# declare-lab/tango

Measured on NVIDIA H100. Metric: audio_seconds_per_second, higher is better.
Workload: dtype bf16

## Files before the change

### tango_b200/csrc/attention.cu

```cuda
#include "tng_ptx.cuh"
#include "tng_internal.h"

namespace tng {

constexpr int FA_BM = 128;
constexpr int FA_BN = 64;
constexpr int FA_QCHUNK = FA_BM * 128;
constexpr int FA_KCHUNK = FA_BN * 128;
constexpr int FA_THREADS = 256;

struct AttnParams {
  int Lq, Lk;
  int q_col0, q_lo_off, k_col0, k_lo_off, v_col0, v_lo_off;
  const float* kbias;
  __nv_bfloat16* out;
  long long ld_o;
  int split_off;
  float scale_log2e;
};

template <int D, int DV, int NSPLIT, int NBUF>
struct FlashCfg {
  static constexpr int Q_BYTES = NSPLIT * (D / 64) * FA_QCHUNK;
  static constexpr int K_BYTES = NSPLIT * (D / 64) * FA_KCHUNK;
  static constexpr int V_BYTES = NSPLIT * (DV / 64) * FA_KCHUNK;
  static constexpr int SMEM_BYTES = Q_BYTES + NBUF * (K_BYTES + V_BYTES) + 128;
  static_assert((1 + 4 * NBUF) * 8 <= 128, "the mbarriers fit the 128 bytes after the tiles");
  static_assert(SMEM_BYTES <= 227 * 1024, "an H100 CTA has at most 227 KB of dynamic shared memory");
};

template <int D, int DV, int NSPLIT, int NBUF>
__global__ void __launch_bounds__(FA_THREADS, (D == 64 && NSPLIT == 1) ? 2 : 1)
flash_attention_kernel(const __grid_constant__ CUtensorMap qmap, const __grid_constant__ CUtensorMap kmap,
                       const __grid_constant__ CUtensorMap vmap, const __grid_constant__ AttnParams p) {
  using Cfg = FlashCfg<D, DV, NSPLIT, NBUF>;
  constexpr int DC = D / 64, NV = DV / 64;
  extern __shared__ __align__(1024) uint8_t smem[];
  uint8_t* sQ = smem;
  uint8_t* sK = sQ + Cfg::Q_BYTES;
  uint8_t* sV = sK + NBUF * Cfg::K_BYTES;
  uint64_t* bars = reinterpret_cast<uint64_t*>(sV + NBUF * Cfg::V_BYTES);
  uint64_t* bar_q = bars;
  uint64_t* full_k = bars + 1;
  uint64_t* full_v = bars + 1 + NBUF;
  uint64_t* empty_k = bars + 1 + 2 * NBUF;
  uint64_t* empty_v = bars + 1 + 3 * NBUF;

  const int tid = threadIdx.x;
  const int warp = tid >> 5;
  const int lane = tid & 31;
  const int wg = warp >> 2;
  const int q0 = blockIdx.x * FA_BM;
  const int b = blockIdx.z;
  const int n_tiles = (p.Lk + FA_BN - 1) / FA_BN;
  const int qk_col = blockIdx.y * (DV == D ? D : 0);
  const int vo_col = blockIdx.y * DV;

  auto load_k = [&](int t) {
    const int buf = t % NBUF;
    mbar_arrive_expect_tx(&full_k[buf], Cfg::K_BYTES);
#pragma unroll
    for (int s = 0; s < NSPLIT; ++s)
#pragma unroll
      for (int c = 0; c < DC; ++c)
        tma_load_3d(sK + buf * Cfg::K_BYTES + (s * DC + c) * FA_KCHUNK, &kmap, &full_k[buf],
                    p.k_col0 + s * p.k_lo_off + qk_col + 64 * c, t * FA_BN, b);
  };
  auto load_v = [&](int t) {
    const int buf = t % NBUF;
    mbar_arrive_expect_tx(&full_v[buf], Cfg::V_BYTES);
#pragma unroll
    for (int s = 0; s < NSPLIT; ++s)
#pragma unroll
      for (int c = 0; c < NV; ++c)
        tma_load_3d(sV + buf * Cfg::V_BYTES + (s * NV + c) * FA_KCHUNK, &vmap, &full_v[buf],
                    p.v_col0 + s * p.v_lo_off + vo_col + 64 * c, t * FA_BN, b);
  };

  if (tid == 0) {
    if ((smem_u32(smem) & 1023u) != 0) __trap();
    tma_prefetch_desc(&qmap);
    tma_prefetch_desc(&kmap);
    tma_prefetch_desc(&vmap);
    mbar_init(bar_q, 1);
    for (int i = 0; i < NBUF; ++i) {
      mbar_init(&full_k[i], 1);
      mbar_init(&full_v[i], 1);
      mbar_init(&empty_k[i], 2);
      mbar_init(&empty_v[i], 2);
    }
    fence_mbar_init();
    mbar_arrive_expect_tx(bar_q, Cfg::Q_BYTES);
#pragma unroll
    for (int s = 0; s < NSPLIT; ++s)
#pragma unroll
      for (int c = 0; c < DC; ++c)
        tma_load_3d(sQ + (s * DC + c) * FA_QCHUNK, &qmap, bar_q, p.q_col0 + s * p.q_lo_off + qk_col + 64 * c, q0, b);
    for (int t = 0; t < NBUF && t < n_tiles; ++t) { load_k(t); load_v(t); }
  }
  __syncthreads();

  constexpr int NT = (NSPLIT == 1) ? 1 : 3;
  const int qsel[3] = {0, 1, 0}, ksel[3] = {0, 0, 1};
  const uint32_t q_base = smem_u32(sQ) + wg * (64 * 128);
  const uint32_t k_base = smem_u32(sK), v_base = smem_u32(sV);
  const float sc = p.scale_log2e;
  constexpr float LOG2E = 1.4426950408889634f;
  const float* kb = p.kbias ? p.kbias + static_cast<long long>(b) * p.Lk : nullptr;
  const int t4 = lane & 3;
  float m_run[2] = {-INFINITY, -INFINITY};
  float l_run[2] = {0.f, 0.f};
  float o[NV][32];
#pragma unroll
  for (int n = 0; n < NV; ++n)
#pragma unroll
    for (int i = 0; i < 32; ++i) o[n][i] = 0.f;

  mbar_wait(bar_q, 0);
  for (int t = 0; t < n_tiles; ++t) {
    const int buf = t % NBUF;
    const uint32_t ph = (t / NBUF) & 1;
    if (NBUF > 1 && tid == 0 && t >= 1 && t - 1 + NBUF < n_tiles) {
      const int pb = (t - 1) % NBUF;
      const uint32_t pph = ((t - 1) / NBUF) & 1;
      mbar_wait(&empty_k[pb], pph);
      load_k(t - 1 + NBUF);
      mbar_wait(&empty_v[pb], pph);
      load_v(t - 1 + NBUF);
    }
    float s[32];
    mbar_wait(&full_k[buf], ph);
    fence_regs(s);
    wgmma_fence();
#pragma unroll
    for (int u = 0; u < NT; ++u) {
#pragma unroll
      for (int c = 0; c < DC; ++c) {
        const uint64_t qd = wgmma_desc_sw128(q_base + (qsel[u] * DC + c) * FA_QCHUNK, 16, 1024);
        const uint64_t kd = wgmma_desc_sw128(k_base + buf * Cfg::K_BYTES + (ksel[u] * DC + c) * FA_KCHUNK, 16, 1024);
#pragma unroll
        for (int k = 0; k < 4; ++k) wgmma_ss<64>(s, qd + 2 * k, kd + 2 * k, (u > 0 || c > 0 || k > 0) ? 1u : 0u);
      }
    }
    wgmma_commit();
    wgmma_wait<0>();
    fence_regs(s);
    if ((tid & 127) == 0) mbar_arrive(&empty_k[buf]);
    if (NBUF == 1 && tid == 0 && t + 1 < n_tiles) {
      mbar_wait(&empty_k[buf], ph);
      load_k(t + 1);
    }

    const int kv0 = t * FA_BN;
    const bool tail = D == 64 && ((kb != nullptr) || (kv0 + FA_BN > p.Lk));
#pragma unroll
    for (int j = 0; j < 8; ++j) {
#pragma unroll
      for (int e = 0; e < 2; ++e) {
        float bias = 0.f;
        if (tail) {
          const int kv = kv0 + 8 * j + 2 * t4 + e;
          bias = kv < p.Lk ? (kb ? __ldg(kb + kv) * LOG2E : 0.f) : -INFINITY;
        }
        s[4 * j + e] = fmaf(s[4 * j + e], sc, bias);
        s[4 * j + 2 + e] = fmaf(s[4 * j + 2 + e], sc, bias);
      }
    }
    float corr[2];
    softmax_step(s, m_run, l_run, corr);
#pragma unroll
    for (int n = 0; n < NV; ++n) rescale_rows(o[n], corr);
    uint32_t pa[NSPLIT][4][4];
    pack_p(pa[0], s);
    if constexpr (NSPLIT == 2) pack_p<true>(pa[1], s);

    mbar_wait(&full_v[buf], ph);
#pragma unroll
    for (int n = 0; n < NV; ++n) fence_regs(o[n]);
    wgmma_fence();
#pragma unroll
    for (int u = 0; u < NT; ++u) {
      const int ps = (NSPLIT == 2 && u == 1) ? NSPLIT - 1 : 0;
#pragma unroll
      for (int n = 0; n < NV; ++n) {
        const uint64_t vd = wgmma_desc_sw128(v_base + buf * Cfg::V_BYTES + (ksel[u] * NV + n) * FA_KCHUNK, 1024, 1024);
#pragma unroll
        for (int kk = 0; kk < FA_BN / 16; ++kk) wgmma_rs_n64_tb(o[n], pa[ps][kk], vd + ((kk * 2048) >> 4), 1u);
      }
    }
    wgmma_commit();
    wgmma_wait<0>();
#pragma unroll
    for (int n = 0; n < NV; ++n) fence_regs(o[n]);
    if ((tid & 127) == 0) mbar_arrive(&empty_v[buf]);
    if (NBUF == 1 && tid == 0 && t + 1 < n_tiles) {
      mbar_wait(&empty_v[buf], ph);
      load_v(t + 1);
    }
  }

  float inv[2];
  softmax_inv(l_run, inv);
#pragma unroll
  for (int h = 0; h < 2; ++h) {
    const int q = q0 + 64 * wg + 16 * (warp & 3) + (lane >> 2) + 8 * h;
    if (q >= p.Lq) continue;
    __nv_bfloat16* op = p.out + (static_cast<long long>(b) * p.Lq + q) * p.ld_o + vo_col + 2 * t4;
#pragma unroll
    for (int n = 0; n < NV; ++n)
#pragma unroll
      for (int j = 0; j < 8; ++j) {
        const float y0 = o[n][4 * j + 2 * h] * inv[h], y1 = o[n][4 * j + 2 * h + 1] * inv[h];
        *reinterpret_cast<uint32_t*>(op + 64 * n + 8 * j) = pack_bf16(y0, y1);
        if (p.split_off > 0)
          *reinterpret_cast<uint32_t*>(op + p.split_off + 64 * n + 8 * j) = pack_bf16_lo(y0, y1);
      }
  }
}

template <int D, int DV, int NSPLIT, int NBUF>
static int launch_flash(const void* q, long long ld_q, const void* k, long long ld_k, const void* v, long long ld_v,
                        int batch, int ny, const AttnParams& p, const char* what, void* stream) {
  constexpr int smem_bytes = FlashCfg<D, DV, NSPLIT, NBUF>::SMEM_BYTES;
  CUtensorMap qm, km, vm;
  int rc = encode_tmap_rows_bf16(&qm, q, ld_q, p.Lq, batch, FA_BM);
  if (!rc) rc = encode_tmap_rows_bf16(&km, k, ld_k, p.Lk, batch, FA_BN);
  if (!rc) rc = encode_tmap_rows_bf16(&vm, v, ld_v, p.Lk, batch, FA_BN);
  if (!rc) rc = set_max_dynamic_smem<flash_attention_kernel<D, DV, NSPLIT, NBUF>>(smem_bytes, what);
  if (rc) return rc;
  dim3 grid((p.Lq + FA_BM - 1) / FA_BM, ny, batch);
  flash_attention_kernel<D, DV, NSPLIT, NBUF>
      <<<grid, FA_THREADS, smem_bytes, reinterpret_cast<cudaStream_t>(stream)>>>(qm, km, vm, p);
  return check_launch(what);
}

}

using namespace tng;

extern "C" int tng_attention(const tng_attn_desc* d, void* stream) {
  if (!d || !d->q || !d->k || !d->v || !d->out) return set_error(TNG_EINVAL, "attention: null argument");
  if (d->nsplit != 1 && d->nsplit != 2) return set_error(TNG_EINVAL, "attention: nsplit=%d", d->nsplit);
  if (d->batch <= 0 || d->heads <= 0 || d->Lq <= 0 || d->Lk <= 0) return set_error(TNG_EINVAL, "attention: bad sizes");
  if (d->scale <= 0.f) return set_error(TNG_EINVAL, "attention: scale must be positive");
  if (d->ld_o % 8 || d->split_off % 8 || (reinterpret_cast<uintptr_t>(d->out) & 15))
    return set_error(TNG_EINVAL, "attention: output must allow 16-byte stores");
  AttnParams p;
  p.Lq = d->Lq; p.Lk = d->Lk;
  p.q_col0 = d->q_col0; p.q_lo_off = d->q_lo_off;
  p.k_col0 = d->k_col0; p.k_lo_off = d->k_lo_off;
  p.v_col0 = d->v_col0; p.v_lo_off = d->v_lo_off;
  p.kbias = d->kbias;
  p.out = reinterpret_cast<__nv_bfloat16*>(d->out);
  p.ld_o = d->ld_o; p.split_off = d->split_off;
  p.scale_log2e = d->scale * 1.4426950408889634f;
  if (d->nsplit == 2)
    return launch_flash<64, 64, 2, 3>(d->q, d->ld_q, d->k, d->ld_k, d->v, d->ld_v, d->batch, d->heads, p, "attention",
                                      stream);
  return launch_flash<64, 64, 1, 3>(d->q, d->ld_q, d->k, d->ld_k, d->v, d->ld_v, d->batch, d->heads, p, "attention",
                                    stream);
}

extern "C" int tng_attention_wide(const void* q, int64_t ld_q, int32_t q_col0, const void* k, int64_t ld_k, int32_t k_col0,
                                  const void* v, int64_t ld_v, int32_t v_col0, void* out, int64_t ld_o, int32_t batch,
                                  int32_t L, int32_t dim, float scale, void* stream) {
  if (!q || !k || !v || !out || batch <= 0 || L <= 0) return set_error(TNG_EINVAL, "attention_wide: bad argument");
  if (dim != 512) return set_error(TNG_EINVAL, "attention_wide: head width %d unsupported (512 only)", dim);
  if (L % FA_BM != 0) return set_error(TNG_EINVAL, "attention_wide: L = %d must be a multiple of %d", L, FA_BM);
  if (scale <= 0.f) return set_error(TNG_EINVAL, "attention_wide: scale must be positive");
  if (ld_o % 8 || (reinterpret_cast<uintptr_t>(out) & 15)) return set_error(TNG_EINVAL, "attention_wide: output must allow 16-byte stores");
  AttnParams p{};
  p.Lq = L; p.Lk = L;
  p.q_col0 = q_col0; p.k_col0 = k_col0; p.v_col0 = v_col0;
  p.out = reinterpret_cast<__nv_bfloat16*>(out);
  p.ld_o = ld_o;
  p.scale_log2e = scale * 1.4426950408889634f;
  return launch_flash<512, 256, 1, 1>(q, ld_q, k, ld_k, v, ld_v, batch, 2, p, "attention_wide", stream);
}
```

### tango_b200/csrc/tng_ptx.cuh

```cuda
#pragma once
#include <cuda_runtime.h>
#include <cuda_bf16.h>
#include <cuda.h>
#include <stdint.h>
#include <stdio.h>
#include "../../include/tango_b200.h"

namespace tng {

#ifndef TNG_SPIN_LIMIT
#define TNG_SPIN_LIMIT (1u << 28)
#endif

__device__ __forceinline__ uint32_t smem_u32(const void* p) {
  return static_cast<uint32_t>(__cvta_generic_to_shared(p));
}

__device__ __forceinline__ void mbar_init(uint64_t* bar, uint32_t count) {
  asm volatile("mbarrier.init.shared::cta.b64 [%0], %1;" ::"r"(smem_u32(bar)), "r"(count));
}
__device__ __forceinline__ void fence_mbar_init() {
  asm volatile("fence.mbarrier_init.release.cluster;" ::: "memory");
}
__device__ __forceinline__ void mbar_arrive_expect_tx(uint64_t* bar, uint32_t bytes) {
  asm volatile("mbarrier.arrive.expect_tx.shared::cta.b64 _, [%0], %1;" ::"r"(smem_u32(bar)), "r"(bytes)
               : "memory");
}
__device__ __forceinline__ void mbar_arrive(uint64_t* bar) {
  asm volatile("mbarrier.arrive.shared::cta.b64 _, [%0];" ::"r"(smem_u32(bar)) : "memory");
}
__device__ __forceinline__ void mbar_arrive_if(uint64_t* bar, bool pred) {
  asm volatile(
      "{\n\t.reg .pred p;\n\tsetp.ne.b32 p, %1, 0;\n\t@p mbarrier.arrive.shared::cta.b64 _, [%0];\n\t}"
      ::"r"(smem_u32(bar)), "r"((uint32_t)pred) : "memory");
}
template <int N>
__device__ __forceinline__ void setmaxnreg_dec() { asm volatile("setmaxnreg.dec.sync.aligned.u32 %0;" ::"n"(N)); }
template <int N>
__device__ __forceinline__ void setmaxnreg_inc() { asm volatile("setmaxnreg.inc.sync.aligned.u32 %0;" ::"n"(N)); }
__device__ __forceinline__ uint32_t mbar_try_wait(uint64_t* bar, uint32_t parity) {
  uint32_t ok;
  asm volatile(
      "{\n\t"
      ".reg .pred P;\n\t"
      "mbarrier.try_wait.parity.shared::cta.b64 P, [%1], %2;\n\t"
      "selp.u32 %0, 1, 0, P;\n\t"
      "}\n"
      : "=r"(ok)
      : "r"(smem_u32(bar)), "r"(parity)
      : "memory");
  return ok;
}
__device__ __forceinline__ void mbar_wait(uint64_t* bar, uint32_t parity) {
  uint32_t spins = 0;
  while (!mbar_try_wait(bar, parity)) {
    if (++spins > TNG_SPIN_LIMIT) __trap();
  }
}

__device__ __forceinline__ void tma_prefetch_desc(const CUtensorMap* m) {
  asm volatile("prefetch.tensormap [%0];" ::"l"(reinterpret_cast<uint64_t>(m)) : "memory");
}
__device__ __forceinline__ void tma_load_2d(void* smem, const CUtensorMap* m, uint64_t* bar, int c0, int c1) {
  asm volatile(
      "cp.async.bulk.tensor.2d.shared::cluster.global.mbarrier::complete_tx::bytes [%0], [%1, {%3, %4}], [%2];"
      ::"r"(smem_u32(smem)), "l"(reinterpret_cast<uint64_t>(m)), "r"(smem_u32(bar)), "r"(c0), "r"(c1)
      : "memory");
}
__device__ __forceinline__ void tma_load_3d(void* smem, const CUtensorMap* m, uint64_t* bar, int c0, int c1,
                                            int c2) {
  asm volatile(
      "cp.async.bulk.tensor.3d.shared::cluster.global.mbarrier::complete_tx::bytes [%0], [%1, {%3, %4, %5}], [%2];"
      ::"r"(smem_u32(smem)), "l"(reinterpret_cast<uint64_t>(m)), "r"(smem_u32(bar)), "r"(c0), "r"(c1), "r"(c2)
      : "memory");
}
__device__ __forceinline__ void tma_load_4d(void* smem, const CUtensorMap* m, uint64_t* bar, int c0, int c1,
                                            int c2, int c3) {
  asm volatile(
      "cp.async.bulk.tensor.4d.shared::cluster.global.mbarrier::complete_tx::bytes [%0], [%1, {%3, %4, %5, %6}], "
      "[%2];" ::"r"(smem_u32(smem)),
      "l"(reinterpret_cast<uint64_t>(m)), "r"(smem_u32(bar)), "r"(c0), "r"(c1), "r"(c2), "r"(c3)
      : "memory");
}

__device__ __forceinline__ void wgmma_fence() { asm volatile("wgmma.fence.sync.aligned;" ::: "memory"); }
__device__ __forceinline__ void wgmma_commit() { asm volatile("wgmma.commit_group.sync.aligned;" ::: "memory"); }
template <int N>
__device__ __forceinline__ void wgmma_wait() {
  asm volatile("wgmma.wait_group.sync.aligned %0;" ::"n"(N) : "memory");
}
template <int R>
__device__ __forceinline__ void fence_regs(float (&d)[R]) {
#pragma unroll
  for (int i = 0; i < R; ++i) asm volatile("" : "+f"(d[i])::"memory");
}

__device__ __forceinline__ uint64_t wgmma_desc_sw128(uint32_t saddr, uint32_t lbo_bytes, uint32_t sbo_bytes) {
  uint64_t d = 0;
  d |= static_cast<uint64_t>((saddr & 0x3FFFF) >> 4);
  d |= static_cast<uint64_t>((lbo_bytes >> 4) & 0x3FFF) << 16;
  d |= static_cast<uint64_t>((sbo_bytes >> 4) & 0x3FFF) << 32;
  d |= static_cast<uint64_t>(1) << 62;
  return d;
}

template <int N>
__device__ __forceinline__ void wgmma_ss(float (&d)[N / 2], uint64_t a_desc, uint64_t b_desc, uint32_t scale_d);

template <>
__device__ __forceinline__ void wgmma_ss<32>(float (&d)[16], uint64_t a_desc, uint64_t b_desc, uint32_t scale_d) {
  asm volatile(
      "{\n\t.reg .pred p;\n\tsetp.ne.b32 p, %18, 0;\n\t"
      "wgmma.mma_async.sync.aligned.m64n32k16.f32.bf16.bf16 {%0, %1, %2, %3, %4, %5, %6, %7, %8, %9, %10, %11, %12, %13, %14, %15}, %16, %17, p, 1, 1, 0, 0;\n\t}\n"
      : "+f"(d[0]), "+f"(d[1]), "+f"(d[2]), "+f"(d[3]), "+f"(d[4]), "+f"(d[5]), "+f"(d[6]), "+f"(d[7]),
        "+f"(d[8]), "+f"(d[9]), "+f"(d[10]), "+f"(d[11]), "+f"(d[12]), "+f"(d[13]), "+f"(d[14]), "+f"(d[15])
      : "l"(a_desc), "l"(b_desc), "r"(scale_d));
}

template <>
__device__ __forceinline__ void wgmma_ss<64>(float (&d)[32], uint64_t a_desc, uint64_t b_desc, uint32_t scale_d) {
  asm volatile(
      "{\n\t.reg .pred p;\n\tsetp.ne.b32 p, %34, 0;\n\t"
      "wgmma.mma_async.sync.aligned.m64n64k16.f32.bf16.bf16 {%0, %1, %2, %3, %4, %5, %6, %7, %8, %9, %10, %11, %12, %13, %14, %15, %16, %17, %18, %19, %20, %21, %22, %23, %24, %25, %26, %27, %28, %29, %30, %31}, %32, %33, p, 1, 1, 0, 0;\n\t}\n"
      : "+f"(d[0]), "+f"(d[1]), "+f"(d[2]), "+f"(d[3]), "+f"(d[4]), "+f"(d[5]), "+f"(d[6]), "+f"(d[7]),
        "+f"(d[8]), "+f"(d[9]), "+f"(d[10]), "+f"(d[11]), "+f"(d[12]), "+f"(d[13]), "+f"(d[14]), "+f"(d[15]),
        "+f"(d[16]), "+f"(d[17]), "+f"(d[18]), "+f"(d[19]), "+f"(d[20]), "+f"(d[21]), "+f"(d[22]), "+f"(d[23]),
        "+f"(d[24]), "+f"(d[25]), "+f"(d[26]), "+f"(d[27]), "+f"(d[28]), "+f"(d[29]), "+f"(d[30]), "+f"(d[31])
      : "l"(a_desc), "l"(b_desc), "r"(scale_d));
}

template <>
__device__ __forceinline__ void wgmma_ss<128>(float (&d)[64], uint64_t a_desc, uint64_t b_desc, uint32_t scale_d) {
  asm volatile(
      "{\n\t.reg .pred p;\n\tsetp.ne.b32 p, %66, 0;\n\t"
      "wgmma.mma_async.sync.aligned.m64n128k16.f32.bf16.bf16 {%0, %1, %2, %3, %4, %5, %6, %7, %8, %9, %10, %11, %12, %13, %14, %15, %16, %17, %18, %19, %20, %21, %22, %23, %24, %25, %26, %27, %28, %29, %30, %31, %32, %33, %34, %35, %36, %37, %38, %39, %40, %41, %42, %43, %44, %45, %46, %47, %48, %49, %50, %51, %52, %53, %54, %55, %56, %57, %58, %59, %60, %61, %62, %63}, %64, %65, p, 1, 1, 0, 0;\n\t}\n"
      : "+f"(d[0]), "+f"(d[1]), "+f"(d[2]), "+f"(d[3]), "+f"(d[4]), "+f"(d[5]), "+f"(d[6]), "+f"(d[7]),
        "+f"(d[8]), "+f"(d[9]), "+f"(d[10]), "+f"(d[11]), "+f"(d[12]), "+f"(d[13]), "+f"(d[14]), "+f"(d[15]),
        "+f"(d[16]), "+f"(d[17]), "+f"(d[18]), "+f"(d[19]), "+f"(d[20]), "+f"(d[21]), "+f"(d[22]), "+f"(d[23]),
        "+f"(d[24]), "+f"(d[25]), "+f"(d[26]), "+f"(d[27]), "+f"(d[28]), "+f"(d[29]), "+f"(d[30]), "+f"(d[31]),
        "+f"(d[32]), "+f"(d[33]), "+f"(d[34]), "+f"(d[35]), "+f"(d[36]), "+f"(d[37]), "+f"(d[38]), "+f"(d[39]),
        "+f"(d[40]), "+f"(d[41]), "+f"(d[42]), "+f"(d[43]), "+f"(d[44]), "+f"(d[45]), "+f"(d[46]), "+f"(d[47]),
        "+f"(d[48]), "+f"(d[49]), "+f"(d[50]), "+f"(d[51]), "+f"(d[52]), "+f"(d[53]), "+f"(d[54]), "+f"(d[55]),
        "+f"(d[56]), "+f"(d[57]), "+f"(d[58]), "+f"(d[59]), "+f"(d[60]), "+f"(d[61]), "+f"(d[62]), "+f"(d[63])
      : "l"(a_desc), "l"(b_desc), "r"(scale_d));
}

template <>
__device__ __forceinline__ void wgmma_ss<160>(float (&d)[80], uint64_t a_desc, uint64_t b_desc, uint32_t scale_d) {
  asm volatile(
      "{\n\t.reg .pred p;\n\tsetp.ne.b32 p, %82, 0;\n\t"
      "wgmma.mma_async.sync.aligned.m64n160k16.f32.bf16.bf16 {%0, %1, %2, %3, %4, %5, %6, %7, %8, %9, %10, %11, %12, %13, %14, %15, %16, %17, %18, %19, %20, %21, %22, %23, %24, %25, %26, %27, %28, %29, %30, %31, %32, %33, %34, %35, %36, %37, %38, %39, %40, %41, %42, %43, %44, %45, %46, %47, %48, %49, %50, %51, %52, %53, %54, %55, %56, %57, %58, %59, %60, %61, %62, %63, %64, %65, %66, %67, %68, %69, %70, %71, %72, %73, %74, %75, %76, %77, %78, %79}, %80, %81, p, 1, 1, 0, 0;\n\t}\n"
      : "+f"(d[0]), "+f"(d[1]), "+f"(d[2]), "+f"(d[3]), "+f"(d[4]), "+f"(d[5]), "+f"(d[6]), "+f"(d[7]),
        "+f"(d[8]), "+f"(d[9]), "+f"(d[10]), "+f"(d[11]), "+f"(d[12]), "+f"(d[13]), "+f"(d[14]), "+f"(d[15]),
        "+f"(d[16]), "+f"(d[17]), "+f"(d[18]), "+f"(d[19]), "+f"(d[20]), "+f"(d[21]), "+f"(d[22]), "+f"(d[23]),
        "+f"(d[24]), "+f"(d[25]), "+f"(d[26]), "+f"(d[27]), "+f"(d[28]), "+f"(d[29]), "+f"(d[30]), "+f"(d[31]),
        "+f"(d[32]), "+f"(d[33]), "+f"(d[34]), "+f"(d[35]), "+f"(d[36]), "+f"(d[37]), "+f"(d[38]), "+f"(d[39]),
        "+f"(d[40]), "+f"(d[41]), "+f"(d[42]), "+f"(d[43]), "+f"(d[44]), "+f"(d[45]), "+f"(d[46]), "+f"(d[47]),
        "+f"(d[48]), "+f"(d[49]), "+f"(d[50]), "+f"(d[51]), "+f"(d[52]), "+f"(d[53]), "+f"(d[54]), "+f"(d[55]),
        "+f"(d[56]), "+f"(d[57]), "+f"(d[58]), "+f"(d[59]), "+f"(d[60]), "+f"(d[61]), "+f"(d[62]), "+f"(d[63]),
        "+f"(d[64]), "+f"(d[65]), "+f"(d[66]), "+f"(d[67]), "+f"(d[68]), "+f"(d[69]), "+f"(d[70]), "+f"(d[71]),
        "+f"(d[72]), "+f"(d[73]), "+f"(d[74]), "+f"(d[75]), "+f"(d[76]), "+f"(d[77]), "+f"(d[78]), "+f"(d[79])
      : "l"(a_desc), "l"(b_desc), "r"(scale_d));
}

template <>
__device__ __forceinline__ void wgmma_ss<256>(float (&d)[128], uint64_t a_desc, uint64_t b_desc, uint32_t scale_d) {
  asm volatile(
      "{\n\t.reg .pred p;\n\tsetp.ne.b32 p, %130, 0;\n\t"
      "wgmma.mma_async.sync.aligned.m64n256k16.f32.bf16.bf16 {%0, %1, %2, %3, %4, %5, %6, %7, %8, %9, %10, %11, %12, %13, %14, %15, %16, %17, %18, %19, %20, %21, %22, %23, %24, %25, %26, %27, %28, %29, %30, %31, %32, %33, %34, %35, %36, %37, %38, %39, %40, %41, %42, %43, %44, %45, %46, %47, %48, %49, %50, %51, %52, %53, %54, %55, %56, %57, %58, %59, %60, %61, %62, %63, %64, %65, %66, %67, %68, %69, %70, %71, %72, %73, %74, %75, %76, %77, %78, %79, %80, %81, %82, %83, %84, %85, %86, %87, %88, %89, %90, %91, %92, %93, %94, %95, %96, %97, %98, %99, %100, %101, %102, %103, %104, %105, %106, %107, %108, %109, %110, %111, %112, %113, %114, %115, %116, %117, %118, %119, %120, %121, %122, %123, %124, %125, %126, %127}, %128, %129, p, 1, 1, 0, 0;\n\t}\n"
      : "+f"(d[0]), "+f"(d[1]), "+f"(d[2]), "+f"(d[3]), "+f"(d[4]), "+f"(d[5]), "+f"(d[6]), "+f"(d[7]),
        "+f"(d[8]), "+f"(d[9]), "+f"(d[10]), "+f"(d[11]), "+f"(d[12]), "+f"(d[13]), "+f"(d[14]), "+f"(d[15]),
        "+f"(d[16]), "+f"(d[17]), "+f"(d[18]), "+f"(d[19]), "+f"(d[20]), "+f"(d[21]), "+f"(d[22]), "+f"(d[23]),
        "+f"(d[24]), "+f"(d[25]), "+f"(d[26]), "+f"(d[27]), "+f"(d[28]), "+f"(d[29]), "+f"(d[30]), "+f"(d[31]),
        "+f"(d[32]), "+f"(d[33]), "+f"(d[34]), "+f"(d[35]), "+f"(d[36]), "+f"(d[37]), "+f"(d[38]), "+f"(d[39]),
        "+f"(d[40]), "+f"(d[41]), "+f"(d[42]), "+f"(d[43]), "+f"(d[44]), "+f"(d[45]), "+f"(d[46]), "+f"(d[47]),
        "+f"(d[48]), "+f"(d[49]), "+f"(d[50]), "+f"(d[51]), "+f"(d[52]), "+f"(d[53]), "+f"(d[54]), "+f"(d[55]),
        "+f"(d[56]), "+f"(d[57]), "+f"(d[58]), "+f"(d[59]), "+f"(d[60]), "+f"(d[61]), "+f"(d[62]), "+f"(d[63]),
        "+f"(d[64]), "+f"(d[65]), "+f"(d[66]), "+f"(d[67]), "+f"(d[68]), "+f"(d[69]), "+f"(d[70]), "+f"(d[71]),
        "+f"(d[72]), "+f"(d[73]), "+f"(d[74]), "+f"(d[75]), "+f"(d[76]), "+f"(d[77]), "+f"(d[78]), "+f"(d[79]),
        "+f"(d[80]), "+f"(d[81]), "+f"(d[82]), "+f"(d[83]), "+f"(d[84]), "+f"(d[85]), "+f"(d[86]), "+f"(d[87]),
        "+f"(d[88]), "+f"(d[89]), "+f"(d[90]), "+f"(d[91]), "+f"(d[92]), "+f"(d[93]), "+f"(d[94]), "+f"(d[95]),
        "+f"(d[96]), "+f"(d[97]), "+f"(d[98]), "+f"(d[99]), "+f"(d[100]), "+f"(d[101]), "+f"(d[102]), "+f"(d[103]),
        "+f"(d[104]), "+f"(d[105]), "+f"(d[106]), "+f"(d[107]), "+f"(d[108]), "+f"(d[109]), "+f"(d[110]), "+f"(d[111]),
        "+f"(d[112]), "+f"(d[113]), "+f"(d[114]), "+f"(d[115]), "+f"(d[116]), "+f"(d[117]), "+f"(d[118]), "+f"(d[119]),
        "+f"(d[120]), "+f"(d[121]), "+f"(d[122]), "+f"(d[123]), "+f"(d[124]), "+f"(d[125]), "+f"(d[126]), "+f"(d[127])
      : "l"(a_desc), "l"(b_desc), "r"(scale_d));
}

__device__ __forceinline__ void wgmma_rs_n64_tb(float (&d)[32], const uint32_t (&a)[4], uint64_t b_desc, uint32_t scale_d) {
  asm volatile(
      "{\n\t.reg .pred p;\n\tsetp.ne.b32 p, %37, 0;\n\t"
      "wgmma.mma_async.sync.aligned.m64n64k16.f32.bf16.bf16 {%0, %1, %2, %3, %4, %5, %6, %7, %8, %9, %10, %11, %12, %13, %14, %15, %16, %17, %18, %19, %20, %21, %22, %23, %24, %25, %26, %27, %28, %29, %30, %31}, {%32, %33, %34, %35}, %36, p, 1, 1, 1;\n\t}\n"
      : "+f"(d[0]), "+f"(d[1]), "+f"(d[2]), "+f"(d[3]), "+f"(d[4]), "+f"(d[5]), "+f"(d[6]), "+f"(d[7]),
        "+f"(d[8]), "+f"(d[9]), "+f"(d[10]), "+f"(d[11]), "+f"(d[12]), "+f"(d[13]), "+f"(d[14]), "+f"(d[15]),
        "+f"(d[16]), "+f"(d[17]), "+f"(d[18]), "+f"(d[19]), "+f"(d[20]), "+f"(d[21]), "+f"(d[22]), "+f"(d[23]),
        "+f"(d[24]), "+f"(d[25]), "+f"(d[26]), "+f"(d[27]), "+f"(d[28]), "+f"(d[29]), "+f"(d[30]), "+f"(d[31])
      : "r"(a[0]), "r"(a[1]), "r"(a[2]), "r"(a[3]), "l"(b_desc), "r"(scale_d));
}

__device__ __forceinline__ float ex2_approx(float x) {
  float y;
  asm("ex2.approx.ftz.f32 %0, %1;" : "=f"(y) : "f"(x));
  return y;
}
__device__ __forceinline__ float rcp_approx(float x) {
  float y;
  asm("rcp.approx.ftz.f32 %0, %1;" : "=f"(y) : "f"(x));
  return y;
}
__device__ __forceinline__ float silu_f(float x) {
  return x * rcp_approx(1.0f + ex2_approx(x * -1.4426950408889634f));
}
__device__ __forceinline__ float gelu_erf_f(float x) {
  const float w = fabsf(x) * 0.84932180028801904272f;
  const float t = rcp_approx(fmaf(0.27273748088f, w, 1.0f));
  const float e = ex2_approx(w * -w);
  float poly = fmaf(0.5307027145f, t, -0.7265760135f);
  poly = fmaf(poly, t, 0.7107068705f);
  poly = fmaf(poly, t, -0.142248368f);
  poly = fmaf(poly, t, 0.127414796f);
  const float q = poly * t * e;
  const float phi = x >= 0.0f ? 1.0f - q : q;
  return x * phi;
}
__device__ __forceinline__ float gelu_tanh_f(float x) {
  const float w = x * fmaf(x * x, 0.044715f, 1.0f);
  return x * rcp_approx(1.0f + ex2_approx(w * -2.3022081986f));
}
__device__ __forceinline__ float act_f(float x, int act, float p) {
  if (act == TNG_ACT_SILU) return silu_f(x);
  if (act == TNG_ACT_LRELU) return x > 0.f ? x : x * p;
  return x;
}
__device__ __forceinline__ float warp_sum(float v) {
#pragma unroll
  for (int o = 16; o > 0; o >>= 1) v += __shfl_xor_sync(0xffffffffu, v, o);
  return v;
}
__device__ __forceinline__ float warp_max(float v) {
#pragma unroll
  for (int o = 16; o > 0; o >>= 1) v = fmaxf(v, __shfl_xor_sync(0xffffffffu, v, o));
  return v;
}
__device__ __forceinline__ float quad_sum(float v) {
  v += __shfl_xor_sync(0xffffffffu, v, 1);
  return v + __shfl_xor_sync(0xffffffffu, v, 2);
}
__device__ __forceinline__ float quad_max(float v) {
  v = fmaxf(v, __shfl_xor_sync(0xffffffffu, v, 1));
  return fmaxf(v, __shfl_xor_sync(0xffffffffu, v, 2));
}

__device__ __forceinline__ float bf16_lo(float v) { return v - __bfloat162float(__float2bfloat16_rn(v)); }
__device__ __forceinline__ uint32_t pack_bf16(float a, float b) {
  __nv_bfloat162 v = __floats2bfloat162_rn(a, b);
  return *reinterpret_cast<uint32_t*>(&v);
}
__device__ __forceinline__ uint32_t pack_bf16_lo(float a, float b) { return pack_bf16(bf16_lo(a), bf16_lo(b)); }
__device__ __forceinline__ float4 load_bf16x4(const __nv_bfloat16* p) {
  const uint2 u = *reinterpret_cast<const uint2*>(p);
  const float2 a = __bfloat1622float2(*reinterpret_cast<const __nv_bfloat162*>(&u.x));
  const float2 b = __bfloat1622float2(*reinterpret_cast<const __nv_bfloat162*>(&u.y));
  return make_float4(a.x, a.y, b.x, b.y);
}
__device__ __forceinline__ void store4_bf16(__nv_bfloat16* p, float4 v) {
  uint2 u;
  u.x = pack_bf16(v.x, v.y);
  u.y = pack_bf16(v.z, v.w);
  *reinterpret_cast<uint2*>(p) = u;
}
__device__ __forceinline__ void store4_bf16_lo(__nv_bfloat16* p, float4 v) {
  store4_bf16(p, make_float4(bf16_lo(v.x), bf16_lo(v.y), bf16_lo(v.z), bf16_lo(v.w)));
}
__device__ __forceinline__ void store4_split(__nv_bfloat16* p, float4 v, int split_off) {
  store4_bf16(p, v);
  if (split_off > 0) store4_bf16_lo(p + split_off, v);
}
__device__ __forceinline__ void store_bf16_split(__nv_bfloat16* p, float v, int split_off) {
  const __nv_bfloat16 hi = __float2bfloat16_rn(v);
  *p = hi;
  if (split_off > 0) p[split_off] = __float2bfloat16_rn(v - __bfloat162float(hi));
}

__device__ __forceinline__ void softmax_step(float (&s)[32], float (&m_run)[2], float (&l_run)[2], float (&corr)[2]) {
  float mx[2] = {-INFINITY, -INFINITY};
#pragma unroll
  for (int j = 0; j < 8; ++j) {
#pragma unroll
    for (int e = 0; e < 2; ++e) {
      mx[0] = fmaxf(mx[0], s[4 * j + e]);
      mx[1] = fmaxf(mx[1], s[4 * j + 2 + e]);
    }
  }
  float m_use[2];
#pragma unroll
  for (int h = 0; h < 2; ++h) {
    const float m_new = fmaxf(m_run[h], quad_max(mx[h]));
    m_use[h] = (m_new == -INFINITY) ? 0.f : m_new;
    corr[h] = ex2_approx(m_run[h] - m_use[h]);
    m_run[h] = m_new;
    l_run[h] *= corr[h];
  }
#pragma unroll
  for (int j = 0; j < 8; ++j) {
#pragma unroll
    for (int e = 0; e < 2; ++e) {
      s[4 * j + e] = ex2_approx(s[4 * j + e] - m_use[0]);
      s[4 * j + 2 + e] = ex2_approx(s[4 * j + 2 + e] - m_use[1]);
      l_run[0] += s[4 * j + e];
      l_run[1] += s[4 * j + 2 + e];
    }
  }
}
__device__ __forceinline__ void rescale_rows(float (&o)[32], const float (&corr)[2]) {
#pragma unroll
  for (int j = 0; j < 8; ++j) {
    o[4 * j] *= corr[0]; o[4 * j + 1] *= corr[0];
    o[4 * j + 2] *= corr[1]; o[4 * j + 3] *= corr[1];
  }
}
template <bool LO = false>
__device__ __forceinline__ void pack_p(uint32_t (&pa)[4][4], const float (&s)[32]) {
#pragma unroll
  for (int kk = 0; kk < 4; ++kk)
#pragma unroll
    for (int r = 0; r < 4; ++r) {
      const float x0 = s[8 * kk + 2 * r], x1 = s[8 * kk + 2 * r + 1];
      pa[kk][r] = LO ? pack_bf16_lo(x0, x1) : pack_bf16(x0, x1);
    }
}
__device__ __forceinline__ void softmax_inv(const float (&l_run)[2], float (&inv)[2]) {
#pragma unroll
  for (int h = 0; h < 2; ++h) inv[h] = 1.0f / quad_sum(l_run[h]);
}

}
```

Measured before the change: 12.09.

## Add dedicated TMA producer warp and fold softmax scale into exp argument

For multi-buffered configurations, an extra producer warp now issues the Q/K/V TMA loads and waits on empty barriers, so the consumer warpgroups no longer block on refills inside their loop. For D=64 non-split tiles without bias or tail, the scale multiply is folded into the max and the exp FMA, which saves a pass over the scores. An optional polynomial exp2 emulation is added for offloading work from MUFU, but it is disabled because POLY_EVERY is 0. The extra warp adds register and scheduling pressure and could affect the two-CTA occupancy target.

```diff
diff --git a/tango_b200/csrc/attention.cu b/tango_b200/csrc/attention.cu
--- a/tango_b200/csrc/attention.cu
+++ b/tango_b200/csrc/attention.cu
@@ -7,7 +7,9 @@
 constexpr int FA_BN = 64;
 constexpr int FA_QCHUNK = FA_BM * 128;
 constexpr int FA_KCHUNK = FA_BN * 128;
-constexpr int FA_THREADS = 256;
+constexpr int FA_CONSUMERS = 256;
+constexpr int fa_threads(int nbuf) { return nbuf > 1 ? FA_CONSUMERS + 32 : FA_CONSUMERS; }
+constexpr int FA_POLY_EVERY = 0;
 
 struct AttnParams {
   int Lq, Lk;
@@ -30,7 +32,7 @@
 };
 
 template <int D, int DV, int NSPLIT, int NBUF>
-__global__ void __launch_bounds__(FA_THREADS, (D == 64 && NSPLIT == 1) ? 2 : 1)
+__global__ void __launch_bounds__(fa_threads(NBUF), (D == 64 && NSPLIT == 1) ? 2 : 1)
 flash_attention_kernel(const __grid_constant__ CUtensorMap qmap, const __grid_constant__ CUtensorMap kmap,
                        const __grid_constant__ CUtensorMap vmap, const __grid_constant__ AttnParams p) {
   using Cfg = FlashCfg<D, DV, NSPLIT, NBUF>;
@@ -77,6 +79,7 @@
                     p.v_col0 + s * p.v_lo_off + vo_col + 64 * c, t * FA_BN, b);
   };
 
+  constexpr bool PRODUCER = NBUF > 1;
   if (tid == 0) {
     if ((smem_u32(smem) & 1023u) != 0) __trap();
     tma_prefetch_desc(&qmap);
@@ -90,15 +93,35 @@
       mbar_init(&empty_v[i], 2);
     }
     fence_mbar_init();
+  }
+  __syncthreads();
+  auto load_q = [&] {
     mbar_arrive_expect_tx(bar_q, Cfg::Q_BYTES);
 #pragma unroll
     for (int s = 0; s < NSPLIT; ++s)
 #pragma unroll
       for (int c = 0; c < DC; ++c)
         tma_load_3d(sQ + (s * DC + c) * FA_QCHUNK, &qmap, bar_q, p.q_col0 + s * p.q_lo_off + qk_col + 64 * c, q0, b);
-    for (int t = 0; t < NBUF && t < n_tiles; ++t) { load_k(t); load_v(t); }
-  }
-  __syncthreads();
+  };
+  if (!PRODUCER && tid == 0) {
+    load_q();
+    load_k(0);
+    load_v(0);
+  }
+
+  if (PRODUCER && tid >= FA_CONSUMERS) {
+    if (tid == FA_CONSUMERS) {
+      load_q();
+      for (int t = 0; t < n_tiles; ++t) {
+        const uint32_t ph = ((t / NBUF) & 1) ^ 1;
+        if (t >= NBUF) mbar_wait(&empty_k[t % NBUF], ph);
+        load_k(t);
+        if (t >= NBUF) mbar_wait(&empty_v[t % NBUF], ph);
+        load_v(t);
+      }
+    }
+    return;
+  }
 
   constexpr int NT = (NSPLIT == 1) ? 1 : 3;
   const int qsel[3] = {0, 1, 0}, ksel[3] = {0, 0, 1};
@@ -120,14 +143,6 @@
   for (int t = 0; t < n_tiles; ++t) {
     const int buf = t % NBUF;
     const uint32_t ph = (t / NBUF) & 1;
-    if (NBUF > 1 && tid == 0 && t >= 1 && t - 1 + NBUF < n_tiles) {
-      const int pb = (t - 1) % NBUF;
-      const uint32_t pph = ((t - 1) / NBUF) & 1;
-      mbar_wait(&empty_k[pb], pph);
-      load_k(t - 1 + NBUF);
-      mbar_wait(&empty_v[pb], pph);
-      load_v(t - 1 + NBUF);
-    }
     float s[32];
     mbar_wait(&full_k[buf], ph);
     fence_regs(s);
@@ -146,28 +161,31 @@
     wgmma_wait<0>();
     fence_regs(s);
     if ((tid & 127) == 0) mbar_arrive(&empty_k[buf]);
-    if (NBUF == 1 && tid == 0 && t + 1 < n_tiles) {
+    if (!PRODUCER && tid == 0 && t + 1 < n_tiles) {
       mbar_wait(&empty_k[buf], ph);
       load_k(t + 1);
     }
 
     const int kv0 = t * FA_BN;
     const bool tail = D == 64 && ((kb != nullptr) || (kv0 + FA_BN > p.Lk));
-#pragma unroll
-    for (int j = 0; j < 8; ++j) {
-#pragma unroll
-      for (int e = 0; e < 2; ++e) {
-        float bias = 0.f;
-        if (tail) {
+    const bool fold = D == 64 && NSPLIT == 1 && !tail;
+    if (tail) {
+#pragma unroll
+      for (int j = 0; j < 8; ++j) {
+#pragma unroll
+        for (int e = 0; e < 2; ++e) {
           const int kv = kv0 + 8 * j + 2 * t4 + e;
-          bias = kv < p.Lk ? (kb ? __ldg(kb + kv) * LOG2E : 0.f) : -INFINITY;
+          const float bias = kv < p.Lk ? (kb ? __ldg(kb + kv) * LOG2E : 0.f) : -INFINITY;
+          s[4 * j + e] = fmaf(s[4 * j + e], sc, bias);
+          s[4 * j + 2 + e] = fmaf(s[4 * j + 2 + e], sc, bias);
         }
-        s[4 * j + e] = fmaf(s[4 * j + e], sc, bias);
-        s[4 * j + 2 + e] = fmaf(s[4 * j + 2 + e], sc, bias);
-      }
+      }
+    } else if (!fold) {
+#pragma unroll
+      for (int i = 0; i < 32; ++i) s[i] = fmaf(s[i], sc, 0.f);
     }
     float corr[2];
-    softmax_step(s, m_run, l_run, corr);
+    softmax_step<(D == 64 && NSPLIT == 1) ? FA_POLY_EVERY : 0>(s, fold ? sc : 1.f, m_run, l_run, corr);
 #pragma unroll
     for (int n = 0; n < NV; ++n) rescale_rows(o[n], corr);
     uint32_t pa[NSPLIT][4][4];
@@ -193,7 +211,7 @@
 #pragma unroll
     for (int n = 0; n < NV; ++n) fence_regs(o[n]);
     if ((tid & 127) == 0) mbar_arrive(&empty_v[buf]);
-    if (NBUF == 1 && tid == 0 && t + 1 < n_tiles) {
+    if (!PRODUCER && tid == 0 && t + 1 < n_tiles) {
       mbar_wait(&empty_v[buf], ph);
       load_v(t + 1);
     }
@@ -230,7 +248,7 @@
   if (rc) return rc;
   dim3 grid((p.Lq + FA_BM - 1) / FA_BM, ny, batch);
   flash_attention_kernel<D, DV, NSPLIT, NBUF>
-      <<<grid, FA_THREADS, smem_bytes, reinterpret_cast<cudaStream_t>(stream)>>>(qm, km, vm, p);
+      <<<grid, fa_threads(NBUF), smem_bytes, reinterpret_cast<cudaStream_t>(stream)>>>(qm, km, vm, p);
   return check_launch(what);
 }
 
diff --git a/tango_b200/csrc/tng_ptx.cuh b/tango_b200/csrc/tng_ptx.cuh
--- a/tango_b200/csrc/tng_ptx.cuh
+++ b/tango_b200/csrc/tng_ptx.cuh
@@ -203,6 +203,16 @@
   asm("ex2.approx.ftz.f32 %0, %1;" : "=f"(y) : "f"(x));
   return y;
 }
+__device__ __forceinline__ float ex2_poly(float x) {
+  x = fmaxf(x, -127.0f);
+  const float t = __fadd_rd(x, 12582912.0f);
+  const float f = x - (t - 12582912.0f);
+  float p = fmaf(0x1.b7ea5cp-7f, f, 0x1.abfe7ep-5f);
+  p = fmaf(p, f, 0x1.ee2374p-3f);
+  p = fmaf(p, f, 0x1.62d6d0p-1f);
+  p = fmaf(p, f, 1.0f);
+  return p * __int_as_float((__float_as_int(t) << 23) + 0x3f800000);
+}
 __device__ __forceinline__ float rcp_approx(float x) {
   float y;
   asm("rcp.approx.ftz.f32 %0, %1;" : "=f"(y) : "f"(x));
@@ -282,7 +292,14 @@
   if (split_off > 0) p[split_off] = __float2bfloat16_rn(v - __bfloat162float(hi));
 }
 
-__device__ __forceinline__ void softmax_step(float (&s)[32], float (&m_run)[2], float (&l_run)[2], float (&corr)[2]) {
+template <int POLY_EVERY = 0>
+__device__ __forceinline__ void softmax_step(float (&s)[32], float scl, float (&m_run)[2], float (&l_run)[2],
+                                             float (&corr)[2]) {
+  auto ex2 = [](float x, int k) {
+    if constexpr (POLY_EVERY > 0)
+      if (k % POLY_EVERY == POLY_EVERY - 1) return ex2_poly(x);
+    return ex2_approx(x);
+  };
   float mx[2] = {-INFINITY, -INFINITY};
 #pragma unroll
   for (int j = 0; j < 8; ++j) {
@@ -295,7 +312,7 @@
   float m_use[2];
 #pragma unroll
   for (int h = 0; h < 2; ++h) {
-    const float m_new = fmaxf(m_run[h], quad_max(mx[h]));
+    const float m_new = fmaxf(m_run[h], quad_max(mx[h]) * scl);
     m_use[h] = (m_new == -INFINITY) ? 0.f : m_new;
     corr[h] = ex2_approx(m_run[h] - m_use[h]);
     m_run[h] = m_new;
@@ -305,8 +322,8 @@
   for (int j = 0; j < 8; ++j) {
 #pragma unroll
     for (int e = 0; e < 2; ++e) {
-      s[4 * j + e] = ex2_approx(s[4 * j + e] - m_use[0]);
-      s[4 * j + 2 + e] = ex2_approx(s[4 * j + 2 + e] - m_use[1]);
+      s[4 * j + e] = ex2(fmaf(s[4 * j + e], scl, -m_use[0]), 2 * j + e);
+      s[4 * j + 2 + e] = ex2(fmaf(s[4 * j + 2 + e], scl, -m_use[1]), 16 + 2 * j + e);
       l_run[0] += s[4 * j + e];
       l_run[1] += s[4 * j + 2 + e];
     }
```

Result: faster. 12.50, median of 6 (+3.4%).
